# wolfcanli/ORB_SLAM2_Modification_with-point-and-line-feature

Measured on AMD Instinct MI355X. Metric: frames/sec (extract+match+pose) at 640x480; ATE RMSE vs ref, higher is better.
Workload: dtype u8

## Files before the change

orb_slam2_modification_with-point-and-line-feature_amd/csrc/orb_extract.hip:

```cpp
#include <hip/hip_runtime.h>
#include <algorithm>
#include <stdint.h>

#include <cstdlib>

#include "orb_geom.h"
#include "orbpl_math.h"
#include "orb_kernels.h"
#include "orbpl_runtime.h"

namespace orbpl {

#include "orb_pattern.inc"
__constant__ int c_pattern[1024];
__constant__ float4 c_pattern_f[256];

__device__ __forceinline__ int reflect101_dev(int p, int len) {
  if (p < 0) p = -p;
  if (p >= len) p = 2 * len - 2 - p;
  return p;
}

__host__ __device__ constexpr int fast_pstride(int win_w) { return (win_w + 7) & ~7; }
__host__ __device__ constexpr int fast_wave_words(int win_w, int win_h) {
  return win_h * (fast_pstride(win_w) / 2) + 4 * win_h;
}

typedef short fshort2 __attribute__((ext_vector_type(2)));
typedef unsigned short fushort2 __attribute__((ext_vector_type(2)));

__device__ __forceinline__ uint32_t umul24(uint32_t a, uint32_t b) {
  return (uint32_t)(uint16_t)a * (uint32_t)(uint16_t)b;
}
template <uint32_t D>
__device__ __forceinline__ uint32_t div_c16(uint32_t i) {
  return umul24(i, (65536u + D - 1) / D) >> 16;
}
__device__ __forceinline__ int imul24(int a, int b) {
  return (int)(int16_t)a * (int)(int16_t)b;
}
__device__ __forceinline__ uint32_t ld_dw(const uint32_t* base, uint32_t dw) {
  return *reinterpret_cast<const uint32_t*>(reinterpret_cast<const char*>(base) + (dw << 2));
}
__device__ __forceinline__ void ld_dw3(const uint32_t* base, uint32_t dw, uint32_t* a, uint32_t* b,
                                       uint32_t* c) {
  const char* p = reinterpret_cast<const char*>(base) + (dw << 2);
  *a = *reinterpret_cast<const uint32_t*>(p);
  *b = *reinterpret_cast<const uint32_t*>(p + 4);
  *c = *reinterpret_cast<const uint32_t*>(p + 8);
}
__device__ __forceinline__ uint32_t ld_b4(const uint8_t* base, uint32_t off) {
  return *reinterpret_cast<const uint32_t*>(base + off);
}
__device__ __forceinline__ void st_b4(uint8_t* base, uint32_t off, uint32_t v) {
  *reinterpret_cast<uint32_t*>(base + off) = v;
}

__device__ __forceinline__ fshort2 as_s2(uint32_t v) { return __builtin_bit_cast(fshort2, v); }
__device__ __forceinline__ fushort2 as_u2(uint32_t v) { return __builtin_bit_cast(fushort2, v); }
__device__ __forceinline__ fshort2 pmin(fshort2 a, fshort2 b) { return __builtin_elementwise_min(a, b); }
__device__ __forceinline__ fshort2 pmax(fshort2 a, fshort2 b) { return __builtin_elementwise_max(a, b); }
__device__ __forceinline__ fushort2 pmaxu(fushort2 a, fushort2 b) { return __builtin_elementwise_max(a, b); }
__device__ __forceinline__ fushort2 pminu(fushort2 a, fushort2 b) { return __builtin_elementwise_min(a, b); }

__device__ __forceinline__ uint32_t ring_pair(const uint2* R, int dy, int dx) {
  const uint32_t j = (uint32_t)(3 + dx);
  return __builtin_amdgcn_perm(R[3 + dy].y, R[3 + dy].x, j | (0x0cu << 8) | ((j + 1) << 16) | (0x0cu << 24));
}

template <bool kMax>
__device__ __forceinline__ void fast_windows(const fushort2* p, fushort2* W) {
  auto op = [](fushort2 a, fushort2 b) { return kMax ? pmaxu(a, b) : pminu(a, b); };
  fushort2 s[2][4], pr[2][4];
#pragma unroll
  for (int h = 0; h < 2; h++) {
    const fushort2* d = p + 8 * h;
    const fushort2 q12 = op(d[1], d[2]), q34 = op(d[3], d[4]), q56 = op(d[5], d[6]);
    s[h][3] = d[7];
    s[h][2] = op(q56, d[7]);
    s[h][1] = op(q34, s[h][2]);
    s[h][0] = op(q12, s[h][1]);
    pr[h][0] = d[0];
// ... 602 lines not shown
          cy = t0 + k;
          py = kEdge - cy;
        } else {
          cy = b0 + (k - nt);
          py = 2 * L.h - 2 - cy + kEdge;
        }
        *so = L.pyr_off + (long long)(cy + kEdge) * L.pitch + 16 * q;
        *dof = L.pyr_off + (long long)py * L.pitch + 16 * q;
      };
      auto mirror_load = [&](int i) __attribute__((always_inline)) -> uint4 {
        long long so, dof;
        mirror_at(min(i, ncopy - 1), &so, &dof);
        return *reinterpret_cast<const uint4*>(fp + so);
      };
      auto mirror_store = [&](int i, uint4 v) __attribute__((always_inline)) {
        if (i >= ncopy) return;
        long long so, dof;
        mirror_at(i, &so, &dof);
        *reinterpret_cast<uint4*>(fp + dof) = v;
      };
      constexpr int T = kPyrThreads;
      for (int i0 = t; i0 < ncopy; i0 += 4 * T) {
        const uint4 v0 = mirror_load(i0), v1 = mirror_load(i0 + T);
        const uint4 v2 = mirror_load(i0 + 2 * T), v3 = mirror_load(i0 + 3 * T);
        mirror_store(i0, v0);
        mirror_store(i0 + T, v1);
        mirror_store(i0 + 2 * T, v2);
        mirror_store(i0 + 3 * T, v3);
      }
    }
    __syncthreads();
    if (stamp) prof[3 + 4 * l] = (long long)wall_clock64();
    pyr_blur_rows(L, fp, bp, B.oa[l], B.ob[l]);
    if (stamp) prof[4 + 4 * l] = (long long)wall_clock64();
  }
}

__device__ __forceinline__ void nms_pair(const uint32_t* M, int ps, int r, int q, fushort2* m,
                                         fushort2* mx) {
  const uint32_t* c = M + r * ps + q;
  *m = as_u2(c[0]);
  fushort2 a = pmaxu(as_u2(c[-1]), as_u2(c[1]));
  a = pmaxu(a, pmaxu(as_u2(c[-ps - 1]), as_u2(c[-ps])));
  a = pmaxu(a, pmaxu(as_u2(c[-ps + 1]), as_u2(c[ps - 1])));
  a = pmaxu(a, pmaxu(as_u2(c[ps]), as_u2(c[ps + 1])));
  *mx = a;
}

__device__ __forceinline__ int wave_incl_scan(int v);

#ifndef ORBPL_FAST_MINW
#define ORBPL_FAST_MINW 6
#endif
#ifndef ORBPL_FAST_DPP
#define ORBPL_FAST_DPP 1
#endif
#ifndef ORBPL_FAST_PREFETCH
#define ORBPL_FAST_PREFETCH 1
#endif
__global__ void __launch_bounds__(256, ORBPL_FAST_MINW) k_fast_cells(const uint8_t* __restrict__ pyr,
                                                    const OrbGeom* __restrict__ g,
                                                    const CellGeom* __restrict__ cells,
                                                    uint32_t* __restrict__ cell_cands,
                                                    int* __restrict__ cell_counts, int ini_th,
                                                    int min_th, int cell0, int cell1) {
  extern __shared__ uint32_t fast_smem[];
  const int wave = __builtin_amdgcn_readfirstlane(threadIdx.x >> 6), lane = threadIdx.x & 63;
  int bx, f;
  xcd_block(&bx, &f);
  const int cell = cell0 + bx * 4 + wave;
  if (cell >= cell1) return;
  const CellGeom cg = cells[cell];
  const int slots = g->cell_slots;
  int* cnt_out = cell_counts + (long long)f * g->ncells_total + cell;
  if (cg.x1 == 0) {
    if (lane == 0) *cnt_out = 0;
    return;
  }
  const int pw = fast_pstride(g->fast_win_w);
  const int pw2 = pw >> 1;
  uint32_t* M = fast_smem + wave * fast_wave_words(g->fast_win_w, g->fast_win_h);
  uint32_t* mask = M + g->fast_win_h * pw2;
  const LevelGeom& L = g->lv[cg.level];
  const int cols = cg.x1 - cg.x0, rows = cg.y1 - cg.y0;
  {
    const int nq = rows * pw2 / 4;
    for (int k = lane; k < nq; k += 64) reinterpret_cast<uint4*>(M)[k] = make_uint4(0, 0, 0, 0);
    for (int k = lane; k < 4 * g->fast_win_h; k += 64) mask[k] = 0;
  }
  __builtin_amdgcn_wave_barrier();
  const int t_ini = max((ini_th < 0 ? 0 : (ini_th > 255 ? 255 : ini_th)) + 1, 2);
  const int t_min = max((min_th < 0 ? 0 : (min_th > 255 ? 255 : min_th)) + 1, 2);
  const int dr = rows - 6, dc = cols - 6;
  const int np = (dc + 1) >> 1;
  const uint32_t inv_np = div_inv(np);
  const int npair = (dr > 0 && dc > 0) ? dr * np : 0;
  uint16_t* M16 = reinterpret_cast<uint16_t*>(M);
  int nseg = 1, rps = dr;
  bool any_ini = false;
  if (npair > 0) {
    nseg = max(1, 64 / np);
    rps = (dr + nseg - 1) / nseg;
    const int seg = div_small(lane, inv_np), p = lane - seg * np;
    const bool in_seg = seg < nseg;
    const int ra = in_seg ? seg * rps : 0, rb = in_seg ? min(ra + rps, dr) : 0;
    const int cx = cg.x0 + 3 + 2 * p;
    const int abase = (cx - 3) & ~3;
    const uint32_t o = (uint32_t)((cx - 3) - abase);
    const uint32_t pitch = (uint32_t)L.pitch;
    const uint8_t* wrow = pyr + (long long)f * g->pyr_bytes + content_off(L, 0, cg.y0);
    const uint32_t acol = (uint32_t)abase;
    const bool has_hi = 2 * p + 1 < dc;
    const bool has_left = p > 0, has_right = p + 1 < np;
    const uint32_t pbit = 1u << p;
    uint2 R[7];
    if (in_seg) {
#pragma unroll
      for (int k = 0; k < 6; k++) R[k + 1] = load_ring_row(wrow, umul24((uint32_t)(ra + k), pitch) + acol, o);
    }
    uint32_t m1 = 0, rmax1 = 0, rmax2 = 0, cmax1 = 0;
    const int nit = __builtin_amdgcn_readfirstlane(rps);
#if ORBPL_FAST_PREFETCH
    uint32_t nw0 = 0, nw1 = 0, nw2 = 0;
    auto ring_raw = [&](int row) __attribute__((always_inline)) {
      const uint8_t* q = wrow + (umul24((uint32_t)row, pitch) + acol);
      nw0 = *reinterpret_cast<const uint32_t*>(q);
      nw1 = *reinterpret_cast<const uint32_t*>(q + 4);
      nw2 = *reinterpret_cast<const uint32_t*>(q + 8);
    };
    if (in_seg && ra < rb) ring_raw(ra + 6);
#endif
    for (int i = 0; i < nit; i++) {
      const int r = ra + i;
      const bool act = r < rb;
      uint32_t m = 0;
      if (act) {
#pragma unroll
        for (int k = 0; k < 6; k++) R[k] = R[k + 1];
#if ORBPL_FAST_PREFETCH
        R[6] = make_uint2(__builtin_amdgcn_alignbyte(nw1, nw0, o), __builtin_amdgcn_alignbyte(nw2, nw1, o));
        if (r + 1 < rb) ring_raw(r + 7);
#else
        R[6] = load_ring_row(wrow, umul24((uint32_t)(r + 6), pitch) + acol, o);
#endif
#if ORBPL_FAST_MM3
        const fshort2 m2 = fast_m2_mm3(R);
#else
        const fshort2 m2 = fast_m2_regs(R);
#endif
        const int wr = r + 3;
        const uint32_t lo = (uint32_t)(uint16_t)m2.x;
        const uint32_t hi = has_hi ? (uint32_t)(uint16_t)m2.y : 0u;
        m = lo | (hi << 16);
        const uint32_t mo = umul24((uint32_t)wr, (uint32_t)pw) + 3 + 2 * p;
        M16[mo] = (uint16_t)lo;
        M16[mo + 1] = (uint16_t)hi;
      }
#if ORBPL_FAST_DPP
      const uint32_t lhi = (uint32_t)__builtin_amdgcn_update_dpp(0, (int)(m >> 16), 0x138, 0xf, 0xf, false);
      const uint32_t rlo = (uint32_t)__builtin_amdgcn_update_dpp(0, (int)(m & 0xFFFFu), 0x130, 0xf, 0xf, false);
#else
      const uint32_t lhi = (uint32_t)__shfl_up((int)(m >> 16), 1, 64);
      const uint32_t rlo = (uint32_t)__shfl_down((int)(m & 0xFFFFu), 1, 64);
#endif
      if (act) {
        const uint32_t Pl = (has_left ? lhi : 0u) | (m << 16);
        const uint32_t Pr = (m >> 16) | ((has_right ? rlo : 0u) << 16);
        const fushort2 cm = pmaxu(as_u2(Pl), as_u2(Pr));
        const uint32_t cmax = __builtin_bit_cast(uint32_t, cm);
        const uint32_t rmax = __builtin_bit_cast(uint32_t, pmaxu(cm, as_u2(m)));
        if (i >= 2) {
          const fushort2 mx = pmaxu(pmaxu(as_u2(rmax2), as_u2(rmax)), as_u2(cmax1));
          const fushort2 mc = as_u2(m1);
          const bool lmax_lo = mc.x > mx.x, lmax_hi = mc.y > mx.y;
          const int row = r - 1;
          uint32_t* mr = mask + 4 * row;
          if (lmax_lo && mc.x >= t_min) atomicOr(mr, pbit);
          if (lmax_hi && mc.y >= t_min) atomicOr(mr + 1, pbit);
          const bool ilo = lmax_lo && mc.x >= t_ini, ihi = lmax_hi && mc.y >= t_ini;
          if (ilo) atomicOr(mr + 2, pbit);
          if (ihi) atomicOr(mr + 3, pbit);
          any_ini |= ilo || ihi;
        }
        rmax2 = rmax1;
        rmax1 = rmax;
        cmax1 = cmax;
        m1 = m;
      }
    }
  }
  __builtin_amdgcn_wave_barrier();
  if (npair > 0) {
    const int nedge = 2 * nseg * np;
    for (int k = lane; k < nedge; k += 64) {
      const int e = div_small(k, inv_np), p = k - e * np;
      const int sg = e >> 1;
      const int ra = sg * rps, rb = min(ra + rps, dr);
      if (ra >= rb) continue;
      const int row = (e & 1) ? rb - 1 : ra;
      if ((e & 1) && rb - 1 == ra) continue;
      fushort2 rm[3], cmc = {0, 0}, m = {0, 0};
#pragma unroll
      for (int d = 0; d < 3; d++) {
        const uint32_t* w = M + (row + 2 + d) * pw2 + 1 + p;
        const uint32_t A = w[0], B = w[1];
        const fushort2 cm = pmaxu(as_u2(A), as_u2(B));
        const fushort2 mm = as_u2(__builtin_amdgcn_perm(B, A, 0x05040302u));
        rm[d] = pmaxu(cm, mm);
        if (d == 1) {
          cmc = cm;
          m = mm;
        }
      }
      const fushort2 mx = pmaxu(pmaxu(rm[0], rm[2]), cmc);
      const bool lmax_lo = m.x > mx.x, lmax_hi = m.y > mx.y;
      const uint32_t pbit = 1u << p;
      uint32_t* mr = mask + 4 * row;
      if (lmax_lo && m.x >= t_min) atomicOr(mr, pbit);
      if (lmax_hi && m.y >= t_min) atomicOr(mr + 1, pbit);
      const bool ilo = lmax_lo && m.x >= t_ini, ihi = lmax_hi && m.y >= t_ini;
      if (ilo) atomicOr(mr + 2, pbit);
      if (ihi) atomicOr(mr + 3, pbit);
      any_ini |= ilo || ihi;
    }
  }
  __builtin_amdgcn_wave_barrier();
  const bool use_ini = __ballot(any_ini) != 0ull;
  const int j0 = use_ini ? 2 : 0;
  uint32_t* out = cell_cands + ((long long)f * g->ncells_total + cell) * slots;
  const int xoff = cg.x0 - kMinBorder, yoff = cg.y0 - kMinBorder;
  uint32_t blo = 0, bhi = 0;
  if (lane < dr && npair > 0) {
    blo = mask[4 * lane + j0];
    bhi = mask[4 * lane + j0 + 1];
  }
  const int cnt = __popc(blo) + __popc(bhi);
  const int incl = wave_incl_scan(cnt);
  const int n = __shfl(incl, 63, 64);
  int pos = incl - cnt;
  const int y = yoff + lane + 3;
  const uint32_t* Mrow = M + (lane + 3) * pw2 + 1;
  uint32_t rem = blo | bhi;
  while (rem) {
    const int p = __builtin_ctz(rem);
    rem &= rem - 1;
    const fushort2 m = as_u2(__builtin_amdgcn_perm(Mrow[p + 1], Mrow[p], 0x05040302u));
    const int x = xoff + 3 + 2 * p;
    if ((blo >> p) & 1u) {
      if (pos < slots) out[pos] = pack_cand(x, y, m.x - 1);
      pos++;
    }
    if ((bhi >> p) & 1u) {
      if (pos < slots) out[pos] = pack_cand(x + 1, y, m.y - 1);
      pos++;
    }
  }
  if (lane == 0) *cnt_out = n < slots ? n : slots;
}

__device__ __forceinline__ int wave_incl_scan(int v) {
  const int lane = threadIdx.x & 63;
#pragma unroll
  for (int o = 1; o < 64; o <<= 1) {
    int u = __shfl_up(v, o, 64);
    if (lane >= o) v += u;
  }
  return v;
}

template <int kPer, int NT = 256>
__device__ int block_excl_scan(int* vals, int n, int* s_wsum) {
  if constexpr (NT == 64) {
    const int lane = threadIdx.x;
    int run = 0;
    for (int base = 0; base < n; base += 64) {
      const int i = base + lane;
      const int v = i < n ? vals[i] : 0;
      const int incl = wave_incl_scan(v);
      if (i < n) vals[i] = run + incl - v;
      run += __shfl(incl, 63, 64);
    }
    __builtin_amdgcn_wave_barrier();
    return run;
  }
  static_assert(NT == 256 || NT == 64, "octree workgroups: 4 waves or 1");
  const int t = threadIdx.x;
  int local[kPer];
  int sum = 0;
#pragma unroll
  for (int k = 0; k < kPer; k++) {
    int i = t * kPer + k;
    local[k] = i < n ? vals[i] : 0;
    sum += local[k];
  }
  int incl = wave_incl_scan(sum);
  const int wave = t >> 6, lane = t & 63;
  if (lane == 63) s_wsum[wave] = incl;
  __syncthreads();
  int wofs = 0, total = 0;
#pragma unroll
  for (int w = 0; w < 4; w++) {
    int s = s_wsum[w];
    if (w < wave) wofs += s;
    total += s;
  }
  int run = wofs + incl - sum;
#pragma unroll
  for (int k = 0; k < kPer; k++) {
    int i = t * kPer + k;
    if (i < n) vals[i] = run;
    run += local[k];
  }
  __syncthreads();
  return total;
}

constexpr int kOctLdsCand = 4096;
#ifndef ORBPL_OCT_WAVE_FROM
#define ORBPL_OCT_WAVE_FROM 3
#endif
constexpr int kOctWaveFrom = ORBPL_OCT_WAVE_FROM;

template <int kCap, int kKn = kOctLdsCand>
struct OctShared {
  uint2 rect[2][kCap];
  int cnt[2][kCap];
  int rank[kCap];
  int upos[kCap];
  int child[4 * kCap];
  int exp_pos[kCap];
  int exp_cnt[kCap];
  int proc[kCap];
  int scan[kOctMaxList];
  int wsum[8];
  int misc[8];
  uint16_t kn[kKn];
};

__device__ __forceinline__ uint2 mk_rect(int x0, int y0, int x1, int y1) {
  return make_uint2((uint32_t)x0 | ((uint32_t)y0 << 16), (uint32_t)x1 | ((uint32_t)y1 << 16));
}

__device__ __forceinline__ int child_of(uint2 r, int x, int y) {
  int x0 = r.x & 0xFFFF, y0 = r.x >> 16, x1 = r.y & 0xFFFF, y1 = r.y >> 16;
  int mx = x0 + ((x1 - x0 + 1) >> 1), my = y0 + ((y1 - y0 + 1) >> 1);
  return x < mx ? (y < my ? 0 : 2) : (y < my ? 1 : 3);
}

__device__ __forceinline__ uint2 child_rect(uint2 r, int c) {
  int x0 = r.x & 0xFFFF, y0 = r.x >> 16, x1 = r.y & 0xFFFF, y1 = r.y >> 16;
  int mx = x0 + ((x1 - x0 + 1) >> 1), my = y0 + ((y1 - y0 + 1) >> 1);
  switch (c) {
    case 0: return mk_rect(x0, y0, mx, my);
    case 1: return mk_rect(mx, y0, x1, my);
    case 2: return mk_rect(x0, my, mx, y1);
    default: return mk_rect(mx, my, x1, y1);
  }
}

__device__ long long g_oct_prof[8 * 16];
__device__ int g_oct_prof_on;

template <int kCap, int NT = 256>
__global__ void __launch_bounds__(NT) k_octree(const OrbGeom* __restrict__ g,
                                                const uint32_t* __restrict__ cell_cands,
                                                const int* __restrict__ cell_counts,
                                                uint32_t* __restrict__ kcand,
                                                int* __restrict__ knode,
                                                uint32_t* __restrict__ kp_list,
                                                int* __restrict__ kp_count,
                                                int* __restrict__ err_flag, int l0) {
  extern __shared__ char smem_raw[];
// ... 549 lines not shown
    kp.size = (float)L.scaled_patch;
    kp.angle = angle;
    kp.response = (float)cand_s(c);
    kp.octave = level;
    kp.class_id = -1;
    out_kps[(long long)f * kp_pitch + opos] = kp;
  }
}

hipError_t upload_pattern(hipStream_t s) {
  static float pf[1024];
  static const bool filled = [] {
    for (int i = 0; i < 1024; i++) pf[i] = (float)bit_pattern_31_[i];
    return true;
  }();
  (void)filled;
  const hipError_t e = hipMemcpyToSymbolAsync(HIP_SYMBOL(c_pattern), bit_pattern_31_,
                                              sizeof(bit_pattern_31_), 0, hipMemcpyHostToDevice, s);
  if (e != hipSuccess) return e;
  return hipMemcpyToSymbolAsync(HIP_SYMBOL(c_pattern_f), pf, sizeof(pf), 0, hipMemcpyHostToDevice, s);
}


int read_od_profile(long long* out8) {
  return hipMemcpyFromSymbol(out8, HIP_SYMBOL(g_od_prof), 6 * sizeof(long long)) == hipSuccess ? 0 : -1;
}

int read_octree_profile(long long* out128) {
  return hipMemcpyFromSymbol(out128, HIP_SYMBOL(g_oct_prof), 128 * sizeof(long long)) == hipSuccess
             ? 0 : -1;
}

void launch_pyramid(const OrbGeom& hg, const OrbGeom* dg, const uint8_t* img, int stride,
                    long long frame_pitch, uint8_t* pyr, uint8_t* blur, const int* rs,
                    const PyrBand* bands, int nbands, int batch, long long* prof, int l0, int l1,
                    hipStream_t s) {
  hipLaunchKernelGGL(k_pyramid, dim3(nbands, batch), dim3(kPyrThreads), 0, s, img, stride,
                     frame_pitch, pyr, blur, dg, rs, bands, prof, l0, l1);
}

void launch_fast(const OrbGeom& hg, const OrbGeom* dg, const CellGeom* cells, const uint8_t* pyr,
                 uint32_t* cell_cands, int* cell_counts, int ini_th, int min_th, int batch,
                 int l0, int l1, hipStream_t s) {
  const size_t smem = 4 * 4 * (size_t)fast_wave_words(hg.fast_win_w, hg.fast_win_h);
  const int c0 = hg.lv[l0].cell_base;
  const int c1 = l1 < hg.nlevels ? hg.lv[l1].cell_base : hg.ncells_total;
  if (c1 <= c0) return;
  hipLaunchKernelGGL(k_fast_cells, dim3((c1 - c0 + 3) / 4, batch), dim3(256), smem, s, pyr, dg,
                     cells, cell_cands, cell_counts, ini_th, min_th, c0, c1);
}

void launch_octree(const OrbGeom& hg, const OrbGeom* dg, const uint32_t* cell_cands,
                   const int* cell_counts, uint32_t* kcand, int* knode, uint32_t* kp_list,
                   int* kp_count, int* err_flag, int batch, int l0, int l1, hipStream_t s) {
  set_smem_attr((const void*)k_octree<1024, 256>, sizeof(OctShared<1024>));
  int cap = 0;
  for (int l = 0; l < hg.nlevels; l++) cap = std::max(cap, hg.lv[l].kp_cap);
  if (once_per_device((const void*)&g_oct_prof_on)) {
    const int on = getenv("ORBPL_OCT_PROFILE") ? 1 : 0;
    (void)hipMemcpyToSymbolAsync(HIP_SYMBOL(g_oct_prof_on), &on, sizeof(int), 0,
                                 hipMemcpyHostToDevice, s);
  }
  const char* wf = getenv("ORBPL_OCT_WAVE_FROM");
  const int wave_from = wf ? atoi(wf) : kOctWaveFrom;
  const bool one_wave = l0 >= wave_from;
#define ORBPL_OCT_LAUNCH(CAP)                                                                   \
  if (one_wave)                                                                                 \
    hipLaunchKernelGGL((k_octree<CAP, 64>), dim3(l1 - l0, batch), dim3(64),                    \
                       sizeof(OctShared<CAP, 2048>), s, dg, cell_cands, cell_counts, kcand,     \
                       knode,                                                                   \
                       kp_list, kp_count, err_flag, l0);                                        \
  else                                                                                          \
    hipLaunchKernelGGL((k_octree<CAP, 256>), dim3(l1 - l0, batch), dim3(256),                  \
                       sizeof(OctShared<CAP>), s, dg, cell_cands, cell_counts, kcand, knode,    \
                       kp_list, kp_count, err_flag, l0);
  if (cap <= 256) {
    ORBPL_OCT_LAUNCH(256)
  } else if (cap <= 512) {
    ORBPL_OCT_LAUNCH(512)
  } else {
    if (one_wave) set_smem_attr((const void*)k_octree<1024, 64>, sizeof(OctShared<1024, 2048>));
    ORBPL_OCT_LAUNCH(1024)
  }
#undef ORBPL_OCT_LAUNCH
}

void launch_orient_desc(const OrbGeom& hg, const OrbGeom* dg, const uint8_t* pyr,
                        const uint8_t* blur, const uint32_t* kp_list, const int* kp_count,
                        orbpl_keypoint_dev* out_kps, uint8_t* out_desc, int kp_pitch, int* out_n,
                        int batch, int l0, int l1, hipStream_t s) {
  const int s0 = hg.lv[l0].kp_base;
  const int s1 = l1 < hg.nlevels ? hg.lv[l1].kp_base : hg.kp_cap_total;
  const int wn = l1 == hg.nlevels ? 1 : 0;
  if (s1 <= s0) return;
  static const char* pe = getenv("ORBPL_OD_PAIR");
  static const bool pair = (pe ? atoi(pe) != 0 : ORBPL_OD_PAIR) && !getenv("ORBPL_OCT_PROFILE");
  if (pair)
    hipLaunchKernelGGL(k_orient_desc2, dim3((s1 - s0 + 7) / 8, batch), dim3(256), 0, s, pyr, blur,
                       dg, kp_list, kp_count, out_kps, out_desc, kp_pitch, out_n, s0, s1, wn);
  else
    hipLaunchKernelGGL(k_orient_desc, dim3((s1 - s0 + 3) / 4, batch), dim3(256), 0, s, pyr, blur,
                       dg, kp_list, kp_count, out_kps, out_desc, kp_pitch, out_n, s0, s1, wn);
}

}
```

orb_slam2_modification_with-point-and-line-feature_amd/csrc/orb_kernels.h:

```cpp
#pragma once
#include <hip/hip_runtime.h>
#include <stdint.h>

#include <vector>

#include "orb_geom.h"

namespace orbpl {

struct orbpl_keypoint_dev {
  float x, y, size, angle, response;
  int octave, class_id;
};

hipError_t upload_pattern(hipStream_t s);
int read_octree_profile(long long* out128);
int read_od_profile(long long* out8);

void launch_pyramid(const OrbGeom& hg, const OrbGeom* dg, const uint8_t* img, int stride,
                    long long frame_pitch, uint8_t* pyr, uint8_t* blur, const int* rs,
                    const PyrBand* bands, int nbands, int batch, long long* prof, int l0, int l1,
                    hipStream_t s);
void launch_fast(const OrbGeom& hg, const OrbGeom* dg, const CellGeom* cells, const uint8_t* pyr,
                 uint32_t* cell_cands, int* cell_counts, int ini_th, int min_th, int batch,
                 int l0, int l1, hipStream_t s);
void launch_octree(const OrbGeom& hg, const OrbGeom* dg, const uint32_t* cell_cands,
                   const int* cell_counts, uint32_t* kcand, int* knode, uint32_t* kp_list,
                   int* kp_count, int* err_flag, int batch, int l0, int l1, hipStream_t s);
void launch_orient_desc(const OrbGeom& hg, const OrbGeom* dg, const uint8_t* pyr,
                        const uint8_t* blur, const uint32_t* kp_list, const int* kp_count,
                        orbpl_keypoint_dev* out_kps, uint8_t* out_desc, int kp_pitch, int* out_n,
                        int batch, int l0, int l1, hipStream_t s);

struct OrbHostGeom {
  OrbGeom g;
  std::vector<CellGeom> cells;
  std::vector<int> rs;
  std::vector<PyrBand> bands;
  std::vector<float> scale, inv_scale, sigma2, inv_sigma2;
};
int build_orb_geometry(int nfeatures, float scale_factor, int nlevels, int W, int H,
                       OrbHostGeom* out, const char** err);

}
```

orb_slam2_modification_with-point-and-line-feature_amd/csrc/orbpl_runtime.cpp:

```cpp
#include <dirent.h>
#include <hip/hip_runtime.h>

#include <cstdio>
#include <cstdlib>
#include <cstring>
#include <unistd.h>
#include <mutex>
#include <map>
#include <set>
#include <cctype>
#include <string>
#include <utility>
#include <vector>

#include "../../include/orbpl.h"
#include "orb_kernels.h"
#include "orbpl_runtime.h"

namespace orbpl {

int g_hw_queues = 4;
int g_runtime_started = 0;
int g_queues_set_by_lib = 0;

// ... 62 lines not shown
  static std::mutex mu;
  static std::set<std::pair<const void*, int>> seen;
  int dev = 0;
  (void)hipGetDevice(&dev);
  std::lock_guard<std::mutex> lk(mu);
  return seen.insert({key, dev}).second;
}

void set_smem_attr(const void* fn, size_t bytes) {
  if (once_per_device(fn))
    (void)hipFuncSetAttribute(fn, hipFuncAttributeMaxDynamicSharedMemorySize, (int)bytes);
}

int device_cu_count() {
  static std::mutex mu;
  static std::map<int, int> cus;
  int dev = 0;
  (void)hipGetDevice(&dev);
  std::lock_guard<std::mutex> lk(mu);
  auto it = cus.find(dev);
  if (it != cus.end()) return it->second;
  int n = 0;
  if (hipDeviceGetAttribute(&n, hipDeviceAttributeMultiprocessorCount, dev) != hipSuccess || n <= 0)
    n = 256;
  cus[dev] = n;
  return n;
}

}

using namespace orbpl;

struct orbx_ctx {
  orbpl_orb_params params{};
  int device = 0;
  int max_batch = 0;
  OrbHostGeom hg;
  hipStream_t stream = nullptr;
  hipEvent_t ev[6] = {};
  hipStream_t fstream = nullptr;
  hipEvent_t ev_group[kMaxLevels] = {};
  hipEvent_t ev_fjoin = nullptr;
  hipEvent_t ev_kern[kKernelBrackets] = {};
  int ngroups = 1;
  int group_end[kMaxLevels] = {};
  bool timed = false;
  OrbGeom* d_geom = nullptr;
  CellGeom* d_cells = nullptr;
  int* d_rs = nullptr;
  PyrBand* d_bands = nullptr;
  long long* d_pyr_prof = nullptr;
  int pyr_bands = 0;
  int group_bands[kFastGroups] = {0, 0, 0, 0};
  uint8_t* d_in = nullptr;
  uint8_t* d_pyr = nullptr;
  uint8_t* d_blur = nullptr;
  uint32_t* d_cell_cands = nullptr;
  int* d_cell_counts = nullptr;
  uint32_t* d_kcand = nullptr;
  int* d_knode = nullptr;
  uint32_t* d_kp_list = nullptr;
  int* d_kp_count = nullptr;
  orbpl_keypoint_dev* d_out_kps = nullptr;
  uint8_t* d_out_desc = nullptr;
  int* d_out_n = nullptr;
  int* d_err = nullptr;
  int last_batch = 0;
};

#define HIP_CHECK(expr)                                              \
  do {                                                               \
    hipError_t _e = (expr);                                          \
    if (_e != hipSuccess) return orbpl::hip_fail(_e, #expr, __LINE__); \
  } while (0)

extern "C" {

const char* orbpl_last_error(void) { return orbpl::g_last_error.c_str(); }

const char* orbpl_version(void) { return "orbpl gfx950 r4"; }

int orbpl_hw_queue_state(int* queues, int* runtime_started, int* set_by_library,
                         int* lsd_split_1024) {
  if (queues) *queues = orbpl::g_hw_queues;
  if (runtime_started) *runtime_started = orbpl::g_runtime_started;
  if (set_by_library) *set_by_library = orbpl::g_queues_set_by_lib;
  if (lsd_split_1024) *lsd_split_1024 = orbpl::lsd_split_decision(1024) ? 1 : 0;
  return ORBPL_OK;
}

int orbpl_device_count(int* n) {
  if (!n) return arg_fail("n is NULL");
  int c = 0;
  hipError_t e = hipGetDeviceCount(&c);
  if (e != hipSuccess) {
    *n = 0;
    hip_fail(e, "hipGetDeviceCount", __LINE__);
    return ORBPL_ERR_NODEVICE;
  }
  *n = c;
  return c > 0 ? ORBPL_OK : ORBPL_ERR_NODEVICE;
}

int orbpl_dev_malloc(int device, int64_t bytes, void** out) {
  if (!out || bytes < 0) return arg_fail("bad argument");
  HIP_CHECK(hipSetDevice(device));
// ... 145 lines not shown
    c->group_end[c->ngroups++] = nl;
    if (c->ngroups > 1) {
      CK(hipStreamCreateWithFlags(&c->fstream, hipStreamNonBlocking));
      for (int i = 0; i < c->ngroups; i++)
        CK(hipEventCreateWithFlags(&c->ev_group[i], hipEventDisableTiming));
      CK(hipEventCreateWithFlags(&c->ev_fjoin, hipEventDisableTiming));
    }
  }
  const size_t B = (size_t)max_batch;
  CK(hipMalloc(&c->d_geom, sizeof(OrbGeom)));
  CK(hipMalloc(&c->d_cells, sizeof(CellGeom) * std::max<size_t>(1, c->hg.cells.size())));
  CK(hipMalloc(&c->d_rs, sizeof(int) * c->hg.rs.size()));
  CK(hipMalloc(&c->d_bands, sizeof(PyrBand) * c->hg.bands.size()));
  CK(hipMalloc(&c->d_in, B * (size_t)width * height));
  CK(hipMalloc(&c->d_pyr, B * (size_t)g.pyr_bytes));
  CK(hipMalloc(&c->d_blur, B * (size_t)g.blur_bytes));
  CK(hipMalloc(&c->d_cell_cands, B * (size_t)std::max(1, g.ncells_total) * g.cell_slots * 4));
  CK(hipMalloc(&c->d_cell_counts, B * (size_t)std::max(1, g.ncells_total) * 4));
  CK(hipMalloc(&c->d_kcand, B * (size_t)std::max(1, g.cand_cap_total) * 4));
  CK(hipMalloc(&c->d_knode, B * (size_t)std::max(1, g.cand_cap_total) * 4));
  CK(hipMalloc(&c->d_kp_list, B * (size_t)g.kp_cap_total * 4));
  CK(hipMalloc(&c->d_kp_count, B * (size_t)g.nlevels * 4));
  CK(hipMalloc(&c->d_out_kps, B * (size_t)g.kp_cap_total * sizeof(orbpl_keypoint_dev)));
  CK(hipMalloc(&c->d_out_desc, B * (size_t)g.kp_cap_total * 32));
  CK(hipMalloc(&c->d_out_n, B * 4));
  CK(hipMalloc(&c->d_err, 4));
  CK(hipMemsetAsync(c->d_err, 0, 4, c->stream));
  CK(hipMemsetAsync(c->d_pyr, 0, B * (size_t)g.pyr_bytes, c->stream));
  CK(hipMemsetAsync(c->d_blur, 0, B * (size_t)g.blur_bytes, c->stream));
  CK(hipMemcpyAsync(c->d_geom, &g, sizeof(OrbGeom), hipMemcpyHostToDevice, c->stream));
  if (!c->hg.cells.empty())
    CK(hipMemcpyAsync(c->d_cells, c->hg.cells.data(), sizeof(CellGeom) * c->hg.cells.size(),
                      hipMemcpyHostToDevice, c->stream));
  CK(hipMemcpyAsync(c->d_rs, c->hg.rs.data(), sizeof(int) * c->hg.rs.size(), hipMemcpyHostToDevice,
                    c->stream));
  CK(hipMemcpyAsync(c->d_bands, c->hg.bands.data(), sizeof(PyrBand) * c->hg.bands.size(),
                    hipMemcpyHostToDevice, c->stream));
  if (const char* e = getenv("ORBPL_PYR_BANDS")) {
    const int b = atoi(e);
    if (b == 1 || b == 2 || b == 4 || b == 8) c->pyr_bands = b;
  }
  if (const char* e = getenv("ORBPL_PYR_GROUP_BANDS")) {
    int gi = 0;
    for (const char* q = e; *q && gi < kFastGroups;) {
      if (!isdigit((unsigned char)*q)) {
        q++;
        continue;
      }
      const int b = atoi(q);
      while (isdigit((unsigned char)*q)) q++;
      c->group_bands[gi++] = (b == 1 || b == 2 || b == 4 || b == 8) ? b : 0;
    }
  }
  if (getenv("ORBPL_PYR_PROFILE")) {
    CK(hipMalloc(&c->d_pyr_prof, 8 * (1 + 4 * kMaxLevels)));
    CK(hipMemsetAsync(c->d_pyr_prof, 0, 8 * (1 + 4 * kMaxLevels), c->stream));
  }
  CK(upload_pattern(c->stream));
  CK(hipStreamSynchronize(c->stream));
#undef CK
  *out = c;
  return ORBPL_OK;
}

int orbx_debug_pyr_profile(orbx_ctx* c, long long* out, int cap, int* n) {
  if (!c || !out || !n) return arg_fail("bad argument");
  if (!c->d_pyr_prof) return arg_fail("ORBPL_PYR_PROFILE was not set when the context was created");
  HIP_CHECK(hipStreamSynchronize(c->stream));
  const int L = c->hg.g.nlevels;
  std::vector<long long> p(1 + 4 * kMaxLevels);
  HIP_CHECK(hipMemcpy(p.data(), c->d_pyr_prof, p.size() * 8, hipMemcpyDeviceToHost));
  *n = std::min(cap, 4 * L);
  for (int i = 0; i < *n; i++) out[i] = (p[i + 1] - p[i]) * 10;
  return ORBPL_OK;
}

int orbx_debug_octree_profile(orbx_ctx* c, long long* out128) {
  if (!c || !out128) return arg_fail("bad argument");
  HIP_CHECK(hipStreamSynchronize(c->stream));
  if (read_octree_profile(out128)) return arg_fail("octree profile unavailable");
  for (int l = 0; l < 16; l++)
    for (int k : {0, 1, 2, 3}) out128[8 * l + k] *= 10;
  long long od[6];
  if (read_od_profile(od) == 0)
    for (int k = 0; k < 6; k++) out128[120 + k] = od[k] * 10;
  return ORBPL_OK;
}

int orbx_destroy(orbx_ctx* c) {
  free_ctx(c);
  return ORBPL_OK;
}

int orbx_get_scale_info(const orbx_ctx* c, int* nlevels, float* scale, float* inv_scale,
                        float* sigma2, float* inv_sigma2) {
  if (!c) return arg_fail("NULL ctx");
  const int n = c->hg.g.nlevels;
  if (nlevels) *nlevels = n;
  for (int i = 0; i < n; i++) {
    if (scale) scale[i] = c->hg.scale[i];
    if (inv_scale) inv_scale[i] = c->hg.inv_scale[i];
    if (sigma2) sigma2[i] = c->hg.sigma2[i];
    if (inv_sigma2) inv_sigma2[i] = c->hg.inv_sigma2[i];
  }
  return ORBPL_OK;
}
// ... 24 lines not shown
    if (scale) scale[i] = hg.scale[i];
  }
  if (max_kps) *max_kps = hg.g.kp_cap_total;
  return ORBPL_OK;
}

}

namespace orbpl {
hipStream_t orbx_stream(orbx_ctx* c) { return c->stream; }

constexpr int kLevelPipeMinBatch = 64;

int orbx_run(orbx_ctx* c, const uint8_t* d_imgs, int batch, int stride, long long frame_pitch,
             orbpl_keypoint_dev* d_kps, uint8_t* d_desc, int kp_pitch, int* d_n,
             hipEvent_t* ext_events, hipEvent_t* ext_kernels) {
  const OrbGeom& g = c->hg.g;
  hipStream_t s = c->stream;
  c->timed = ext_events == nullptr;
  hipEvent_t* ev = ext_events ? ext_events : c->ev;
  hipEvent_t* evk = ext_kernels ? ext_kernels : (ext_events ? nullptr : c->ev_kern);
  HIP_CHECK(hipEventRecord(ev[0], s));
  int nb = c->pyr_bands;
  if (!nb) {
    nb = 1;
    while (nb < kPyrMaxBands && nb * batch < 1024) nb *= 2;
  }
  auto bracket = [&](int kind, int gi, int end, hipStream_t st) -> hipError_t {
    return evk ? hipEventRecord(evk[2 * (kind * kFastGroups + gi) + end], st) : hipSuccess;
  };
  const bool pipe = c->ngroups > 1 && batch >= kLevelPipeMinBatch;
  const int ngroups = pipe ? c->ngroups : 1;
  hipStream_t fs = pipe ? c->fstream : s;
  int l0 = 0;
  for (int gi = 0; gi < ngroups; gi++) {
    const int l1 = pipe ? c->group_end[gi] : g.nlevels;
    const int nbg = pipe && c->group_bands[gi] ? c->group_bands[gi] : nb;
    launch_pyramid(g, c->d_geom, d_imgs, stride, frame_pitch, c->d_pyr, c->d_blur, c->d_rs,
                   c->d_bands + pyr_band_base(nbg), nbg, batch, c->d_pyr_prof, l0, l1, s);
    if (pipe) {
      HIP_CHECK(hipEventRecord(c->ev_group[gi], s));
      HIP_CHECK(hipStreamWaitEvent(fs, c->ev_group[gi], 0));
    } else {
      HIP_CHECK(hipEventRecord(ev[1], s));
      HIP_CHECK(hipEventRecord(ev[2], s));
    }
    HIP_CHECK(bracket(0, gi, 0, fs));
    launch_fast(g, c->d_geom, c->d_cells, c->d_pyr, c->d_cell_cands, c->d_cell_counts,
                c->params.ini_th_fast, c->params.min_th_fast, batch, l0, l1, fs);
    HIP_CHECK(bracket(0, gi, 1, fs));
    if (!pipe) HIP_CHECK(hipEventRecord(ev[3], s));
    HIP_CHECK(bracket(1, gi, 0, fs));
    launch_octree(g, c->d_geom, c->d_cell_cands, c->d_cell_counts, c->d_kcand, c->d_knode,
                  c->d_kp_list, c->d_kp_count, c->d_err, batch, l0, l1, fs);
    HIP_CHECK(bracket(1, gi, 1, fs));
    if (!pipe) HIP_CHECK(hipEventRecord(ev[4], s));
    l0 = l1;
  }
  HIP_CHECK(bracket(2, 0, 0, fs));
  launch_orient_desc(g, c->d_geom, c->d_pyr, c->d_blur, c->d_kp_list, c->d_kp_count, d_kps, d_desc,
                     kp_pitch, d_n, batch, 0, g.nlevels, fs);
  HIP_CHECK(bracket(2, 0, 1, fs));
  for (int kind = 0; kind < 3; kind++)
    for (int gi = kind == 2 ? 1 : ngroups; gi < kFastGroups; gi++) {
      HIP_CHECK(bracket(kind, gi, 0, fs));
      HIP_CHECK(bracket(kind, gi, 1, fs));
    }
  if (pipe) {
    HIP_CHECK(hipEventRecord(ev[1], s));
    HIP_CHECK(hipEventRecord(ev[2], s));
    HIP_CHECK(hipEventRecord(c->ev_fjoin, fs));
    HIP_CHECK(hipStreamWaitEvent(s, c->ev_fjoin, 0));
    HIP_CHECK(hipEventRecord(ev[3], s));
    HIP_CHECK(hipEventRecord(ev[4], s));
  }
  HIP_CHECK(hipEventRecord(ev[5], s));
  HIP_CHECK(hipGetLastError());
  c->last_batch = batch;
  return ORBPL_OK;
}
}

extern "C" {

int orbx_synchronize(orbx_ctx* c) {
  if (!c) return arg_fail("NULL ctx");
  HIP_CHECK(hipSetDevice(c->device));
  HIP_CHECK(hipStreamSynchronize(c->stream));
  int flag = 0;
  HIP_CHECK(hipMemcpy(&flag, c->d_err, 4, hipMemcpyDeviceToHost));
  if (flag) {
    HIP_CHECK(hipMemset(c->d_err, 0, 4));
    char buf[128];
    snprintf(buf, sizeof(buf), "kernel capacity overflow (flags 0x%x)", flag);
    orbpl::g_last_error = buf;
    return ORBPL_ERR_OVERFLOW;
  }
  return ORBPL_OK;
}

int orbx_extract(orbx_ctx* c, const uint8_t* img, int width, int height, int stride,
                 orbpl_keypoint* kps, uint8_t* desc, int cap, int* n) {
  if (!c || !n) return arg_fail("NULL argument");
  *n = 0;
  if (!img || width <= 0 || height <= 0) return ORBPL_OK;
  if (width != c->hg.g.W || height != c->hg.g.H)
    return arg_fail("image size differs from the size given to orbx_create");
// ... 137 lines not shown
```

Measured before the change: 128,000.

## Restructure FAST NMS into ballot threshold pass with lazy min-threshold fallback

Replaces the streaming per-row non-max suppression with atomics and edge fixups. Each row now ballots which scores pass the initial threshold and writes bitmasks. A second pass runs the 3x3 max test only on set bits, and the full min-threshold NMS runs only when no cell candidate passes the initial threshold. It also moves the octree one-wave level cutoff env read from per-launch to context creation and changes its default so the 64-thread variant is effectively disabled. The prefetch becomes a single 12-byte vector load. This removes LDS atomics and DPP shuffles, at the cost of an extra serial bit-loop pass and a possible second sweep over sparse cells.

Result: faster. 130,700 (median of 6 runs) (+2.1%).

```diff
diff --git a/orb_slam2_modification_with-point-and-line-feature_amd/csrc/orb_extract.hip b/orb_slam2_modification_with-point-and-line-feature_amd/csrc/orb_extract.hip
--- a/orb_slam2_modification_with-point-and-line-feature_amd/csrc/orb_extract.hip
+++ b/orb_slam2_modification_with-point-and-line-feature_amd/csrc/orb_extract.hip
@@ -28,6 +28,8 @@
 
 typedef short fshort2 __attribute__((ext_vector_type(2)));
 typedef unsigned short fushort2 __attribute__((ext_vector_type(2)));
+typedef uint32_t fuint3 __attribute__((ext_vector_type(3)));
+typedef fuint3 fuint3_a4 __attribute__((aligned(4)));
 
 __device__ __forceinline__ uint32_t umul24(uint32_t a, uint32_t b) {
   return (uint32_t)(uint16_t)a * (uint32_t)(uint16_t)b;
@@ -736,9 +738,6 @@
 #ifndef ORBPL_FAST_MINW
 #define ORBPL_FAST_MINW 6
 #endif
-#ifndef ORBPL_FAST_DPP
-#define ORBPL_FAST_DPP 1
-#endif
 #ifndef ORBPL_FAST_PREFETCH
 #define ORBPL_FAST_PREFETCH 1
 #endif
@@ -770,7 +769,6 @@
   {
     const int nq = rows * pw2 / 4;
     for (int k = lane; k < nq; k += 64) reinterpret_cast<uint4*>(M)[k] = make_uint4(0, 0, 0, 0);
-    for (int k = lane; k < 4 * g->fast_win_h; k += 64) mask[k] = 0;
   }
   __builtin_amdgcn_wave_barrier();
   const int t_ini = max((ini_th < 0 ? 0 : (ini_th > 255 ? 255 : ini_th)) + 1, 2);
@@ -780,14 +778,20 @@
   const uint32_t inv_np = div_inv(np);
   const int npair = (dr > 0 && dc > 0) ? dr * np : 0;
   uint16_t* M16 = reinterpret_cast<uint16_t*>(M);
-  int nseg = 1, rps = dr;
-  bool any_ini = false;
+  const int nseg = npair > 0 ? max(1, 64 / np) : 1;
+  const int rps = (dr + nseg - 1) / nseg;
+  const int seg = div_small(lane, inv_np), p = lane - seg * np;
+  const bool in_seg = npair > 0 && seg < nseg;
+  const int ra = in_seg ? seg * rps : 0, rb = in_seg ? min(ra + rps, dr) : 0;
+  const int nit = __builtin_amdgcn_readfirstlane(rps);
+  const uint32_t npmask = np > 0 ? (1u << np) - 1u : 0u;
+  auto store_row_bits = [&](int r, bool act, unsigned long long blo, unsigned long long bhi)
+      __attribute__((always_inline)) {
+    if (act && p == 0)
+      *reinterpret_cast<uint2*>(mask + 4 * r) =
+          make_uint2((uint32_t)(blo >> lane) & npmask, (uint32_t)(bhi >> lane) & npmask);
+  };
   if (npair > 0) {
-    nseg = max(1, 64 / np);
-    rps = (dr + nseg - 1) / nseg;
-    const int seg = div_small(lane, inv_np), p = lane - seg * np;
-    const bool in_seg = seg < nseg;
-    const int ra = in_seg ? seg * rps : 0, rb = in_seg ? min(ra + rps, dr) : 0;
     const int cx = cg.x0 + 3 + 2 * p;
     const int abase = (cx - 3) & ~3;
     const uint32_t o = (uint32_t)((cx - 3) - abase);
@@ -795,22 +799,16 @@
     const uint8_t* wrow = pyr + (long long)f * g->pyr_bytes + content_off(L, 0, cg.y0);
     const uint32_t acol = (uint32_t)abase;
     const bool has_hi = 2 * p + 1 < dc;
-    const bool has_left = p > 0, has_right = p + 1 < np;
-    const uint32_t pbit = 1u << p;
+    const uint32_t t_ini_hi = (uint32_t)t_ini << 16;
     uint2 R[7];
     if (in_seg) {
 #pragma unroll
       for (int k = 0; k < 6; k++) R[k + 1] = load_ring_row(wrow, umul24((uint32_t)(ra + k), pitch) + acol, o);
     }
-    uint32_t m1 = 0, rmax1 = 0, rmax2 = 0, cmax1 = 0;
-    const int nit = __builtin_amdgcn_readfirstlane(rps);
 #if ORBPL_FAST_PREFETCH
-    uint32_t nw0 = 0, nw1 = 0, nw2 = 0;
+    fuint3 nw = {0, 0, 0};
     auto ring_raw = [&](int row) __attribute__((always_inline)) {
-      const uint8_t* q = wrow + (umul24((uint32_t)row, pitch) + acol);
-      nw0 = *reinterpret_cast<const uint32_t*>(q);
-      nw1 = *reinterpret_cast<const uint32_t*>(q + 4);
-      nw2 = *reinterpret_cast<const uint32_t*>(q + 8);
+      nw = *reinterpret_cast<const fuint3_a4*>(wrow + (umul24((uint32_t)row, pitch) + acol));
     };
     if (in_seg && ra < rb) ring_raw(ra + 6);
 #endif
@@ -822,8 +820,8 @@
 #pragma unroll
         for (int k = 0; k < 6; k++) R[k] = R[k + 1];
 #if ORBPL_FAST_PREFETCH
-        R[6] = make_uint2(__builtin_amdgcn_alignbyte(nw1, nw0, o), __builtin_amdgcn_alignbyte(nw2, nw1, o));
-        if (r + 1 < rb) ring_raw(r + 7);
+        R[6] = make_uint2(__builtin_amdgcn_alignbyte(nw.y, nw.x, o), __builtin_amdgcn_alignbyte(nw.z, nw.y, o));
+        ring_raw(min(r + 7, rb + 5));
 #else
         R[6] = load_ring_row(wrow, umul24((uint32_t)(r + 6), pitch) + acol, o);
 #endif
@@ -840,76 +838,57 @@
         M16[mo] = (uint16_t)lo;
         M16[mo + 1] = (uint16_t)hi;
       }
-#if ORBPL_FAST_DPP
-      const uint32_t lhi = (uint32_t)__builtin_amdgcn_update_dpp(0, (int)(m >> 16), 0x138, 0xf, 0xf, false);
-      const uint32_t rlo = (uint32_t)__builtin_amdgcn_update_dpp(0, (int)(m & 0xFFFFu), 0x130, 0xf, 0xf, false);
-#else
-      const uint32_t lhi = (uint32_t)__shfl_up((int)(m >> 16), 1, 64);
-      const uint32_t rlo = (uint32_t)__shfl_down((int)(m & 0xFFFFu), 1, 64);
-#endif
+      store_row_bits(r, act, __ballot((m & 0xFFFFu) >= (uint32_t)t_ini), __ballot(m >= t_ini_hi));
+    }
+  }
+  __builtin_amdgcn_wave_barrier();
+  bool any_ini = false;
+  if (npair > 0) {
+    for (int k = lane; k < 2 * dr; k += 64) {
+      const int row = k >> 1, half = k & 1;
+      uint32_t rem = mask[4 * row + half], keep = 0;
+      const uint16_t* c0 = M16 + umul24((uint32_t)(row + 2), (uint32_t)pw) + 2 + half;
+      while (rem) {
+        const int q = __builtin_ctz(rem);
+        rem &= rem - 1;
+        const uint16_t* c = c0 + 2 * q;
+        const uint32_t up = max(max((uint32_t)c[0], (uint32_t)c[1]), (uint32_t)c[2]);
+        const uint32_t dn = max(max((uint32_t)c[2 * pw], (uint32_t)c[2 * pw + 1]), (uint32_t)c[2 * pw + 2]);
+        const uint32_t mx = max(max(up, dn), max((uint32_t)c[pw], (uint32_t)c[pw + 2]));
+        if ((uint32_t)c[pw + 1] > mx) keep |= 1u << q;
+      }
+      mask[4 * row + 2 + half] = keep;
+      any_ini |= keep != 0;
+    }
+  }
+  const bool use_ini = __ballot(any_ini) != 0ull;
+  if (!use_ini && npair > 0) {
+    for (int i = 0; i < nit; i++) {
+      const int r = ra + i;
+      const bool act = r < rb;
+      bool klo = false, khi = false;
       if (act) {
-        const uint32_t Pl = (has_left ? lhi : 0u) | (m << 16);
-        const uint32_t Pr = (m >> 16) | ((has_right ? rlo : 0u) << 16);
-        const fushort2 cm = pmaxu(as_u2(Pl), as_u2(Pr));
-        const uint32_t cmax = __builtin_bit_cast(uint32_t, cm);
-        const uint32_t rmax = __builtin_bit_cast(uint32_t, pmaxu(cm, as_u2(m)));
-        if (i >= 2) {
-          const fushort2 mx = pmaxu(pmaxu(as_u2(rmax2), as_u2(rmax)), as_u2(cmax1));
-          const fushort2 mc = as_u2(m1);
-          const bool lmax_lo = mc.x > mx.x, lmax_hi = mc.y > mx.y;
-          const int row = r - 1;
-          uint32_t* mr = mask + 4 * row;
-          if (lmax_lo && mc.x >= t_min) atomicOr(mr, pbit);
-          if (lmax_hi && mc.y >= t_min) atomicOr(mr + 1, pbit);
-          const bool ilo = lmax_lo && mc.x >= t_ini, ihi = lmax_hi && mc.y >= t_ini;
-          if (ilo) atomicOr(mr + 2, pbit);
-          if (ihi) atomicOr(mr + 3, pbit);
-          any_ini |= ilo || ihi;
+        fushort2 rm[3], cmc = {0, 0}, m = {0, 0};
+#pragma unroll
+        for (int d = 0; d < 3; d++) {
+          const uint32_t* w = M + (r + 2 + d) * pw2 + 1 + p;
+          const uint32_t A = w[0], B = w[1];
+          const fushort2 cm = pmaxu(as_u2(A), as_u2(B));
+          const fushort2 mm = as_u2(__builtin_amdgcn_perm(B, A, 0x05040302u));
+          rm[d] = pmaxu(cm, mm);
+          if (d == 1) {
+            cmc = cm;
+            m = mm;
+          }
         }
-        rmax2 = rmax1;
-        rmax1 = rmax;
-        cmax1 = cmax;
-        m1 = m;
-      }
+        const fushort2 mx = pmaxu(pmaxu(rm[0], rm[2]), cmc);
+        klo = m.x > mx.x && m.x >= t_min;
+        khi = m.y > mx.y && m.y >= t_min;
+      }
+      store_row_bits(r, act, __ballot(klo), __ballot(khi));
     }
   }
   __builtin_amdgcn_wave_barrier();
-  if (npair > 0) {
-    const int nedge = 2 * nseg * np;
-    for (int k = lane; k < nedge; k += 64) {
-      const int e = div_small(k, inv_np), p = k - e * np;
-      const int sg = e >> 1;
-      const int ra = sg * rps, rb = min(ra + rps, dr);
-      if (ra >= rb) continue;
-      const int row = (e & 1) ? rb - 1 : ra;
-      if ((e & 1) && rb - 1 == ra) continue;
-      fushort2 rm[3], cmc = {0, 0}, m = {0, 0};
-#pragma unroll
-      for (int d = 0; d < 3; d++) {
-        const uint32_t* w = M + (row + 2 + d) * pw2 + 1 + p;
-        const uint32_t A = w[0], B = w[1];
-        const fushort2 cm = pmaxu(as_u2(A), as_u2(B));
-        const fushort2 mm = as_u2(__builtin_amdgcn_perm(B, A, 0x05040302u));
-        rm[d] = pmaxu(cm, mm);
-        if (d == 1) {
-          cmc = cm;
-          m = mm;
-        }
-      }
-      const fushort2 mx = pmaxu(pmaxu(rm[0], rm[2]), cmc);
-      const bool lmax_lo = m.x > mx.x, lmax_hi = m.y > mx.y;
-      const uint32_t pbit = 1u << p;
-      uint32_t* mr = mask + 4 * row;
-      if (lmax_lo && m.x >= t_min) atomicOr(mr, pbit);
-      if (lmax_hi && m.y >= t_min) atomicOr(mr + 1, pbit);
-      const bool ilo = lmax_lo && m.x >= t_ini, ihi = lmax_hi && m.y >= t_ini;
-      if (ilo) atomicOr(mr + 2, pbit);
-      if (ihi) atomicOr(mr + 3, pbit);
-      any_ini |= ilo || ihi;
-    }
-  }
-  __builtin_amdgcn_wave_barrier();
-  const bool use_ini = __ballot(any_ini) != 0ull;
   const int j0 = use_ini ? 2 : 0;
   uint32_t* out = cell_cands + ((long long)f * g->ncells_total + cell) * slots;
   const int xoff = cg.x0 - kMinBorder, yoff = cg.y0 - kMinBorder;
@@ -1001,7 +980,7 @@
 
 constexpr int kOctLdsCand = 4096;
 #ifndef ORBPL_OCT_WAVE_FROM
-#define ORBPL_OCT_WAVE_FROM 3
+#define ORBPL_OCT_WAVE_FROM kMaxLevels
 #endif
 constexpr int kOctWaveFrom = ORBPL_OCT_WAVE_FROM;
 
@@ -1657,7 +1636,8 @@
 
 void launch_octree(const OrbGeom& hg, const OrbGeom* dg, const uint32_t* cell_cands,
                    const int* cell_counts, uint32_t* kcand, int* knode, uint32_t* kp_list,
-                   int* kp_count, int* err_flag, int batch, int l0, int l1, hipStream_t s) {
+                   int* kp_count, int* err_flag, int batch, int l0, int l1, int wave_from,
+                   hipStream_t s) {
   set_smem_attr((const void*)k_octree<1024, 256>, sizeof(OctShared<1024>));
   int cap = 0;
   for (int l = 0; l < hg.nlevels; l++) cap = std::max(cap, hg.lv[l].kp_cap);
@@ -1666,9 +1646,7 @@
     (void)hipMemcpyToSymbolAsync(HIP_SYMBOL(g_oct_prof_on), &on, sizeof(int), 0,
                                  hipMemcpyHostToDevice, s);
   }
-  const char* wf = getenv("ORBPL_OCT_WAVE_FROM");
-  const int wave_from = wf ? atoi(wf) : kOctWaveFrom;
-  const bool one_wave = l0 >= wave_from;
+  const bool one_wave = l0 >= (wave_from >= 0 ? wave_from : kOctWaveFrom);
 #define ORBPL_OCT_LAUNCH(CAP)                                                                   \
   if (one_wave)                                                                                 \
     hipLaunchKernelGGL((k_octree<CAP, 64>), dim3(l1 - l0, batch), dim3(64),                    \
diff --git a/orb_slam2_modification_with-point-and-line-feature_amd/csrc/orb_kernels.h b/orb_slam2_modification_with-point-and-line-feature_amd/csrc/orb_kernels.h
--- a/orb_slam2_modification_with-point-and-line-feature_amd/csrc/orb_kernels.h
+++ b/orb_slam2_modification_with-point-and-line-feature_amd/csrc/orb_kernels.h
@@ -26,7 +26,8 @@
                  int l0, int l1, hipStream_t s);
 void launch_octree(const OrbGeom& hg, const OrbGeom* dg, const uint32_t* cell_cands,
                    const int* cell_counts, uint32_t* kcand, int* knode, uint32_t* kp_list,
-                   int* kp_count, int* err_flag, int batch, int l0, int l1, hipStream_t s);
+                   int* kp_count, int* err_flag, int batch, int l0, int l1, int wave_from,
+                   hipStream_t s);
 void launch_orient_desc(const OrbGeom& hg, const OrbGeom* dg, const uint8_t* pyr,
                         const uint8_t* blur, const uint32_t* kp_list, const int* kp_count,
                         orbpl_keypoint_dev* out_kps, uint8_t* out_desc, int kp_pitch, int* out_n,
diff --git a/orb_slam2_modification_with-point-and-line-feature_amd/csrc/orbpl_runtime.cpp b/orb_slam2_modification_with-point-and-line-feature_amd/csrc/orbpl_runtime.cpp
--- a/orb_slam2_modification_with-point-and-line-feature_amd/csrc/orbpl_runtime.cpp
+++ b/orb_slam2_modification_with-point-and-line-feature_amd/csrc/orbpl_runtime.cpp
@@ -138,6 +138,7 @@
   long long* d_pyr_prof = nullptr;
   int pyr_bands = 0;
   int group_bands[kFastGroups] = {0, 0, 0, 0};
+  int oct_wave_from = -1;
   uint8_t* d_in = nullptr;
   uint8_t* d_pyr = nullptr;
   uint8_t* d_blur = nullptr;
@@ -389,6 +390,7 @@
       c->group_bands[gi++] = (b == 1 || b == 2 || b == 4 || b == 8) ? b : 0;
     }
   }
+  if (const char* e = getenv("ORBPL_OCT_WAVE_FROM")) c->oct_wave_from = std::max(0, atoi(e));
   if (getenv("ORBPL_PYR_PROFILE")) {
     CK(hipMalloc(&c->d_pyr_prof, 8 * (1 + 4 * kMaxLevels)));
     CK(hipMemsetAsync(c->d_pyr_prof, 0, 8 * (1 + 4 * kMaxLevels), c->stream));
@@ -519,7 +521,8 @@
     if (!pipe) HIP_CHECK(hipEventRecord(ev[3], s));
     HIP_CHECK(bracket(1, gi, 0, fs));
     launch_octree(g, c->d_geom, c->d_cell_cands, c->d_cell_counts, c->d_kcand, c->d_knode,
-                  c->d_kp_list, c->d_kp_count, c->d_err, batch, l0, l1, fs);
+                  c->d_kp_list, c->d_kp_count, c->d_err, batch, l0, l1, c->oct_wave_from,
+                  fs);
     HIP_CHECK(bracket(1, gi, 1, fs));
     if (!pipe) HIP_CHECK(hipEventRecord(ev[4], s));
     l0 = l1;
```
